# hsiehScalAR/KNODE-Cosserat

Measured on AMD Instinct MI355X. Metric: rod-steps/sec (N=100 segments, batch=1024), higher is better.
Workload: dtype f64

## Files before the change

knode-cosserat_amd/csrc/kr_mso_impl.hpp:

```cpp
#pragma once
#include "kr_ms_impl.hpp"

namespace kr {

constexpr int MSO_B0 = 7 + 17 * (MS_P - 1);
#ifndef KR_MSO_LAG
#define KR_MSO_LAG 1
#endif
constexpr int MSO_LAG = KR_MSO_LAG;
static_assert(MSO_B0 + MS_P <= WAVE, "the verifying lanes must fit beside the forward-difference lanes");

template <typename T, int HS>
__host__ __device__ inline size_t mso_lds_elems(int N) {
  return ms_lds_elems<T, HS>(N, true, false) + 80;
}

__device__ __forceinline__ void wave_sync_lds() {
  __builtin_amdgcn_fence(__ATOMIC_ACQ_REL, "wavefront");
  __builtin_amdgcn_wave_barrier();
}

#define KR_LDS __attribute__((address_space(3)))
template <typename T, int NV>
__device__ __forceinline__ void lds_load_vec(const T* src, T (&v)[NV]) {
  using V = typename Vec16<T>::type;
  constexpr int n = Vec16<T>::n;
  static_assert(NV % n == 0, "vector load needs a multiple of 16 bytes");
  const KR_LDS V* s = (const KR_LDS V*)src;
#pragma unroll
  for (int c = 0; c < NV / n; ++c) {
    const V x = s[c];
#pragma unroll
    for (int e = 0; e < n; ++e) v[c * n + e] = x[e];
  }
}
template <typename T, int NV>
__device__ __forceinline__ void lds_store_vec(T* dst, const T (&v)[NV]) {
  using V = typename Vec16<T>::type;
  constexpr int n = Vec16<T>::n;
  static_assert(NV % n == 0, "vector store needs a multiple of 16 bytes");
  KR_LDS V* d = (KR_LDS V*)dst;
#pragma unroll
  for (int c = 0; c < NV / n; ++c) {
    V x;
#pragma unroll
    for (int e = 0; e < n; ++e) x[e] = v[c * n + e];
    d[c] = x;
  }
}

template <typename U>
__device__ __forceinline__ U own_sgpr(U v) {
  asm volatile("" : "+s"(v));
  return v;
}

template <typename U>
__device__ __forceinline__ U* own_sgpr_global(U* p) {
  uintptr_t v = (uintptr_t)p;
  asm volatile("" : "+s"(v));
  return (U*)(__attribute__((address_space(1))) U*)v;
}

#ifdef KR_MS_STAMPS
struct MsoStats { unsigned long long total = 0, sweeps = 0, merged = 0, quick = 0, chord = 0, rejects = 0, retries = 0, rebuilds = 0, t_sweep = 0, t_alg = 0, t_pred = 0, t_verdict = 0, t_cond = 0, t_fin = 0, t_upd = 0, t_v1 = 0, t_v2 = 0, t_c1 = 0, t_c2 = 0, t_copy = 0; };
#endif

template <typename T, bool DIAG, int HS, int OCC = 1, typename PSRC = RodConst<T>>
__global__ __launch_bounds__(WAVE * MS_WPB, OCC) void mso_sim_kernel(const PSRC Pa, const SimArgs<T> A) {
  extern __shared__ __attribute__((aligned(16))) unsigned char smem_raw[];
  const int N = rod_src_N<T>(Pa);
  const int lane = threadIdx.x & (WAVE - 1);
  const int wv = threadIdx.x / WAVE;
  const int64_t rod = (int64_t)blockIdx.x * MS_WPB + wv;
  if (rod >= A.B) return;
  const auto& Pc = rod_src_row<T>(Pa, rod);
  const size_t rod_elems = (size_t)N * KR_SLOTS;
  T* const a_states = own_sgpr_global(A.states);
  const int64_t a_slot_elems = own_sgpr(A.slot_elems);
  const int a_ring = own_sgpr(A.ring);
  T* const a_tip = own_sgpr_global(A.tip);
  int32_t* const a_status = own_sgpr_global(A.status);
  const int a_residual_test = own_sgpr(A.residual_test), a_predictor = own_sgpr(A.predictor);
  const T hc1 = own_sgpr(A.hc1), hc2 = own_sgpr(A.hc2);
  const int T_steps = own_sgpr((int)A.T_steps);
  const MsLds<T> L = ms_carve<T, HS>(reinterpret_cast<T*>(smem_raw) + (size_t)wv * mso_lds_elems<T, HS>(N), N, true, false);
  T* const Es = L.Es;
  T* const XB = L.XB;
  T* const Tm = L.Tm;
  T* const X0 = L.Xs;
  const ptrdiff_t X_d = (L.c12 + (size_t)N * 12) - L.Xs;
  int xsel = 0;
  T* Xs = X0;
  T* XsB = X0 + X_d;
  T* const EsB = Es + MSO_B0 * MS_YP;
  const MsRole R = ms_role(lane, N);
  const int iv = R.iv, col = R.col;
  const bool isA = lane < MSO_B0;
  const bool isB = lane >= MSO_B0 && lane < MSO_B0 + MS_P;
  const int ib = isB ? lane - MSO_B0 : 0;
  const int s_l = isB ? ms_interval_start(ib, R.sbase, R.srem) : R.s_i;
  const int len_l = isB ? R.sbase + (ib < R.srem ? 1 : 0) : R.len_i;
  ms_cold_fill<T>(rod_src_mem<T>(Pa, rod), L.cold, lane);
  wave_sync();

  auto slot_ptr = [&](int slot) -> T* { return a_states + (int64_t)slot * a_slot_elems + rod * rod_elems; };
  auto state_ptr = [&](int k) -> T* { return slot_ptr(a_ring ? k % 3 : k); };
  T* const lead0 = L.c12;
  const ptrdiff_t lead_d = L.hist - L.c12;
  auto lead_of = [&](int t) -> T* { return lead0 + (ptrdiff_t)(t & 1) * lead_d; };
  auto rebuild = [&](int t) {
    const T* cur = state_ptr(t);
    const T* prv = t > 0 ? state_ptr(t - 1) : (A.prev_init ? A.prev_init + rod * rod_elems : cur);
    T* const lc = lead_of(t);
    T* const lp = lead_of(t - 1);
    for (int j = lane; j < N; j += WAVE) {
      T cv[12], pv[12];
      load_hist_vec<T, 12>(cur + (size_t)j * KR_SLOTS, cv);
      load_hist_vec<T, 12>(prv + (size_t)j * KR_SLOTS, pv);
      lds_store_vec<T, 12>(lc + (size_t)j * 12, cv);
      lds_store_vec<T, 12>(lp + (size_t)j * 12, pv);
    }
    wave_sync();
  };
  const T* ctl = A.ctl + rod * A.T_steps * 4;
  auto load_fc = [&](int t) -> V3<T> {
    V3<T> tf{T(0), T(0), T(0)};
#pragma unroll
    for (int k = 0; k < 4; ++k) {
      const T tt = ctl[(size_t)t * 4 + k];
      tf.x += tt * L.cold[CD_TDIRS + k * 3 + 0];
      tf.y += tt * L.cold[CD_TDIRS + k * 3 + 1];
      tf.z += tt * L.cold[CD_TDIRS + k * 3 + 2];
    }
    return {L.cold[CD_RHOAG] + tf.x, L.cold[CD_RHOAG + 1] + tf.y, L.cold[CD_RHOAG + 2] + tf.z};
  };

  const T* s0 = state_ptr(0);
  const T* sp0 = A.prev_init ? A.prev_init + rod * rod_elems : s0;
  MsPred<T> Q;
  double* img = A.pred_io ? A.pred_io + (size_t)rod * MS_PRED_ROWS * WAVE : nullptr;
  if (img && A.pred_load) ms_pred_load<T>(Q, img, lane);
  else ms_pred_init<T>(Q, lane, R, s0, sp0, A.prev_init != nullptr, a_predictor);
  V3<T> vlast, ulast;
  {
    const T* cl = s0 + (size_t)(N - 1) * KR_SLOTS;
    vlast = {cl[SL_V], cl[SL_V + 1], cl[SL_V + 2]};
    ulast = {cl[SL_U], cl[SL_U + 1], cl[SL_U + 2]};
  }
  const T tol = own_sgpr(A.tol), tolA = own_sgpr(A.tolA), fd_eps = own_sgpr(A.fd_eps);
  const int maxit = own_sgpr(A.maxit);
  T kappa = Q.kappa;
  T Gguess = lane < 6 ? A.G[rod * 6 + lane] : T(0);
  MsStamps stamps;
#ifdef KR_MS_STAMPS
  MsoStats st;
  unsigned long long t_begin, tq;
  KR_STAMP(t_begin);
  tq = t_begin;
#endif

  rebuild(0);

  int tA = 0;
  int rsA = 0;
  bool merged = false;
  int it = 0;
  int order = Q.next_order;
  bool retried = false;
  T dn_prev = T(-1);
  bool have_fac = false, below = false;
  float amp = -1.f;
  T dnB = T(-1);
  float ampB = -1.f;
  bool belowB = false;
  int itB = 0, orderB = 0;
  bool pred_skip = false;
  bool reverify = false;
  int resume_at = T_steps;
  T Xreg[MS_P - 1][2];
#pragma unroll
  for (int g = 0; g < MS_P - 1; ++g) Xreg[g][0] = Xreg[g][1] = T(0);
  V3<T> fcA = load_fc(0), fcB = fcA;
  V3<T> fcN = load_fc(T_steps > 1 ? 1 : 0);
  static_assert(DIAG, "the in-sweep history record assumes diagonal material matrices");
  T hk_a[3], hk_b[3], hk_c[3];
#pragma unroll
  for (int c = 0; c < 3; ++c) {
    hk_a[c] = L.cold[CD_KSEI + 4 * c] * L.cold[CD_KSEV + c];
    hk_b[c] = -L.cold[CD_KSEI + 4 * c] * L.cold[CD_BSE + 4 * c];
    hk_c[c] = -L.cold[CD_KBTI + 4 * c] * L.cold[CD_BBT + 4 * c];
  }

  ms_pred_guess<T>(Q, order, lane, L.cold, Xs);
  wave_sync_lds();
  if (order <= 0 && lane < 6) Xs[0 * MS_YP + 7 + lane] = Gguess;
  wave_sync_lds();

  struct Upd { T updP, updG, xsP, xsG, xsY[MS_P - 1]; };

  while (true) {
    const bool runA = tA < T_steps;
    const int tB = tA - 1;
    T yr[19];
    {
      const T* src = isB ? XsB + ib * MS_YP : Xs + iv * MS_YP;
#pragma unroll
      for (int q = 0; q < 19; ++q) yr[q] = src[q];
    }
    const T hstep = (isA && col > 0) ? fd_eps * fmax(fabs(Xs[iv * MS_YP + (R.comp > 0 ? R.comp : 3)]), T(1)) : T(1);
    int comp = R.comp;
    asm volatile("" : "+v"(comp));
#pragma unroll
    for (int q = 3; q < 19; ++q) yr[q] += q == comp ? hstep : T(0);
    RodState<T> y = rows_to_state(yr);
    const V3<T> fc = isB ? fcB : fcA;
    const int lag = (isA && merged) ? MSO_LAG : 0;
    const bool act = isB ? merged : (isA && runA);
    const int trips = R.lmax + ((merged && runA) ? MSO_LAG : 0);
    T* const out_rod = slot_ptr(rsA);
    auto point_of = [&](int k) -> int {
      const int kk = k - lag;
      return s_l + (kk < 0 ? 0 : (kk < len_l ? kk : len_l - 1));
    };
    const T* const lead_n = lead_of(isB ? tB : tA);
    const T* const lead_o = lead_of(isB ? tB + 1 : tB);
    auto hist_form = [&](const T (&la)[12], const T (&lb)[12]) __attribute__((always_inline)) -> RodHist<T> {
      T raw[12];
#pragma unroll
      for (int c = 0; c < 12; ++c) raw[c] = hc1 * la[c] + hc2 * lb[c];
      RodHist<T> h;
      h.qh = {raw[0], raw[1], raw[2]};
      h.wh = {raw[3], raw[4], raw[5]};
      h.vh = {raw[6], raw[7], raw[8]};
      h.uh = {raw[9], raw[10], raw[11]};
      h.av = {hk_b[0] * raw[6] + hk_a[0], hk_b[1] * raw[7] + hk_a[1], hk_b[2] * raw[8] + hk_a[2]};
      h.au = {hk_c[0] * raw[9], hk_c[1] * raw[10], hk_c[2] * raw[11]};
      return h;
    };
    auto hist_at = [&](int j) __attribute__((always_inline)) -> RodHist<T> {
      T la[12], lb[12];
      lds_load_vec<T, 12>(lead_n + (size_t)j * 12, la);
      lds_load_vec<T, 12>(lead_o + (size_t)j * 12, lb);
      return hist_form(la, lb);
    };
    RodHist<T> hst = hist_at(point_of(0));
    if (!merged) {
      auto fd_point = [&](int j, T dsl) __attribute__((always_inline)) {
        RodState<T> k1;
        V3<T> v, u;
        ode_eval<T, DIAG>(Pc, y, hst, fc, k1, v, u);
        hst = hist_at(j + 1);
        y = state_axpy(y, dsl, k1);
      };
#pragma unroll 2
      for (int t = 0; t < R.sbase; ++t) fd_point(R.s_i + t, Pc.ds);
      if (R.srem) fd_point(R.s_i + (R.len_i > R.sbase ? R.sbase : R.sbase - 1), R.len_i > R.sbase ? Pc.ds : T(0));
    } else {
      const bool lean = a_ring && tB + 4 <= T_steps;
      T* const lead_w = lead_of(tB + 1);
      auto trip = [&](int k, auto full_tag) __attribute__((always_inline)) {
        constexpr bool FULL = decltype(full_tag)::value;
        const int kk = k - lag;
        const bool live = FULL ? act : (act && kk >= 0 && kk < len_l);
        const int j = FULL ? s_l + kk : point_of(k);
        T la[12], lb[12];
        if constexpr (MSO_LAG >= 2) {
          const int jn = FULL ? j + 1 : point_of(k + 1);
          lds_load_vec<T, 12>(lead_n + (size_t)jn * 12, la);
          lds_load_vec<T, 12>(lead_o + (size_t)jn * 12, lb);
        }
        RodState<T> k1;
        V3<T> v, u;
        ode_eval<T, DIAG>(Pc, y, hst, fc, k1, v, u);
        if constexpr (MSO_LAG >= 2) {
          hst = hist_form(la, lb);
          asm volatile("" : "+v"(hst.qh.x), "+v"(hst.qh.y), "+v"(hst.qh.z), "+v"(hst.wh.x), "+v"(hst.wh.y), "+v"(hst.wh.z));
          asm volatile("" : "+v"(hst.vh.x), "+v"(hst.vh.y), "+v"(hst.vh.z), "+v"(hst.uh.x), "+v"(hst.uh.y), "+v"(hst.uh.z));
          asm volatile("" : "+v"(hst.av.x), "+v"(hst.av.y), "+v"(hst.av.z), "+v"(hst.au.x), "+v"(hst.au.y), "+v"(hst.au.z));
        }
        if (isB && live) {
          T rec[KR_SLOTS];
          record_from(y, v, u, rec);
          T lead[12];
#pragma unroll
          for (int c = 0; c < 12; ++c) lead[c] = rec[c];
          if constexpr (FULL) {
            if (!lean) {
              T rest[KR_SLOTS - 12];
#pragma unroll
              for (int c = 0; c < KR_SLOTS - 12; ++c) rest[c] = rec[12 + c];
              store_vec<T, KR_SLOTS - 12>(out_rod + (size_t)j * KR_SLOTS + 12, rest);
            }
          } else {
            store_record(out_rod + (size_t)j * KR_SLOTS, rec);
          }
          lds_store_vec<T, 12>(lead_w + (size_t)j * 12, lead);
        }
        if constexpr (MSO_LAG < 2) hst = hist_at(FULL ? j + 1 : point_of(k + 1));
        const T dsl = live ? Pc.ds : T(0);
        y = state_axpy(y, dsl, k1);
      };
      int k = 0;
      for (; k < MSO_LAG && k < trips; ++k) trip(k, std::false_type{});
#pragma unroll 2
      for (; k < R.sbase; ++k) trip(k, std::true_type{});
      for (; k < trips; ++k) trip(k, std::false_type{});
    }
#ifdef KR_MS_STAMPS
    KR_STAMP_ADD(st.t_sweep, tq);
    st.sweeps += 1;
    if (merged) st.merged += 1;
#endif

    int ln = lane;
    asm volatile("" : "+v"(ln));
    const int kp = ln & 3;
    const int r = 3 + (ln >> 2);
    const bool plane = ln < 3 * (MS_P - 1);
    const int pi = plane ? ln / 3 : 0;
    const int prow = plane ? ln - 3 * pi : 0;
    const bool glane = ln >= WAVE - 6;
    T er[19];
    state_to_rows(y, er);
    T d[6];
    T updY[MS_P - 1];
    T* dYb = XB;
    float dnf = 0.f;
    bool finite = true;
    Upd U;

    auto finish = [&](const T* X, auto base_slot) -> float {
      T* sp = Tm;
      if (kp == 0) {
#pragma unroll
        for (int g = 1; g < MS_P - 1; ++g) dYb[g * MS_YP + r] = updY[g - 1];
      }
      wave_sync_lds();
      if (plane) {
        const int l0 = pi == 0 ? 0 : 7 + 17 * (pi - 1);
        T s = Es[base_slot(pi) * MS_YP + prow] - X[(pi + 1) * MS_YP + prow];
        T av[16], dv[16];
#pragma unroll
        for (int c = 0; c < 16; ++c) {
          const bool use = pi > 0 || c < 6;
          av[c] = use ? Es[(l0 + 1 + c) * MS_YP + prow] : T(0);
          dv[c] = pi > 0 ? dYb[pi * MS_YP + 3 + c] : T(0);
        }
        __builtin_amdgcn_sched_barrier(0);
        T s2 = T(0);
#pragma unroll
        for (int c = 0; c < 16; c += 2) {
          const T da = pi > 0 ? dv[c] : (c < 6 ? d[c < 6 ? c : 0] : T(0));
          const T db = pi > 0 ? dv[c + 1] : (c + 1 < 6 ? d[c + 1 < 6 ? c + 1 : 0] : T(0));
          s = fma(av[c], da, s);
          s2 = fma(av[c + 1], db, s2);
        }
        sp[pi * 3 + prow] = s + s2;
      }
      wave_sync_lds();
      float nf = 0.f;
      U.updP = T(0); U.updG = T(0); U.xsP = T(0); U.xsG = T(0);
      if (plane) {
        U.xsP = X[(pi + 1) * MS_YP + prow];
#pragma unroll
        for (int i = 0; i < MS_P - 1; ++i) {
          const T t = sp[i * 3 + prow];
          U.updP += i <= pi ? t : T(0);
        }
        nf = update_ratio(U.updP, U.xsP);
      }
      if (glane) {
        const int k = ln - (WAVE - 6);
        U.xsG = X[0 * MS_YP + 7 + k];
        U.updG = k == 0 ? d[0] : k == 1 ? d[1] : k == 2 ? d[2] : k == 3 ? d[3] : k == 4 ? d[4] : d[5];
        nf = fmaxf(nf, update_ratio(U.updG, U.xsG));
      }
#pragma unroll
      for (int g = 1; g < MS_P; ++g) {
        U.xsY[g - 1] = T(0);
        if (((g - 1) & 3) == kp) {
          U.xsY[g - 1] = X[g * MS_YP + r];
          nf = fmaxf(nf, update_ratio(updY[g - 1], U.xsY[g - 1]));
        }
      }
      return wave_max_nonneg(nf);
    };
    auto apply = [&](T* X) {
      if (plane) X[(pi + 1) * MS_YP + prow] = U.xsP + U.updP;
      if (glane) X[0 * MS_YP + 7 + (ln - (WAVE - 6))] = U.xsG + U.updG;
#pragma unroll
      for (int g = 1; g < MS_P; ++g)
        if (((g - 1) & 3) == kp) X[g * MS_YP + r] = U.xsY[g - 1] + updY[g - 1];
    };

    if (merged) {
      if (isB) {
#pragma unroll
        for (int q = 0; q < 19; ++q) EsB[ib * MS_YP + q] = er[q];
        if (ib == MS_P - 1) {
          T rec[KR_SLOTS];
          record_from(y, vlast, ulast, rec);
          store_record(out_rod + (size_t)(N - 1) * KR_SLOTS, rec);
          T lead[12];
#pragma unroll
          for (int c = 0; c < 12; ++c) lead[c] = rec[c];
          lds_store_vec<T, 12>(lead_of(tB + 1) + (size_t)(N - 1) * 12, lead);
          if (a_tip) {
            T* tp = a_tip + (rod * T_steps + tB) * 3;
            tp[0] = y.p.x; tp[1] = y.p.y; tp[2] = y.p.z;
          }
        }
      }
      wave_sync_lds();
#ifdef KR_MS_STAMPS
      unsigned long long tv;
      { KR_STAMP(tv); st.t_v1 += tv - tq; }
#endif
      float rn = 0.f;
      if (ln < 3 * MS_YP) {
        const int g = ln / MS_YP, q = ln - MS_YP * g;
        const T x = XsB[(g + 1) * MS_YP + q];
        rn = update_ratio(EsB[g * MS_YP + q] - x, x);
      } else if (ln < 3 * MS_YP + 6) {
        const int k = ln - 3 * MS_YP;
        const T e = EsB[(MS_P - 1) * MS_YP + 7 + k];
        rn = update_ratio(L.cold[CD_FTIP + k] - e, e);
      }
      rn = wave_max_nonneg(rn);
#ifdef KR_MS_STAMPS
      KR_STAMP_ADD(st.t_v2, tv);
#endif
      const float est = ampB * rn;
      bool accepted = a_residual_test != 0 && ampB > 0.f && T(256) * (T)est <= tol;
      float dnv = est;
#ifdef KR_MS_STAMPS
      if (accepted) st.quick += 1;
#endif
      if (!accepted) {
        T* ach = XB;
        T* rt = XB + 4 * MS_YP;
        dYb = XB + MS_YP * 8;
        T areg[MS_P - 1];
        areg[0] = EsB[0 * MS_YP + r] - XsB[1 * MS_YP + r];
        if (kp == 0) ach[1 * MS_YP + r] = areg[0];
        wave_sync_lds();
#pragma unroll
        for (int g = 1; g < MS_P; ++g) {
          const int l0 = 7 + 17 * (g - 1);
          T av[4], xv[4];
#pragma unroll
          for (int cc = 0; cc < 4; ++cc) {
            av[cc] = Es[(l0 + 1 + 4 * kp + cc) * MS_YP + r];
            xv[cc] = ach[g * MS_YP + 3 + 4 * kp + cc];
          }
          const T e0 = EsB[g * MS_YP + r];
          const T ynext = g < MS_P - 1 ? XsB[(g + 1) * MS_YP + r] : T(0);
          T part = fma(av[0], xv[0], av[1] * xv[1]) + fma(av[2], xv[2], av[3] * xv[3]);
          part += quad_xor<0xB1>(part);
          part += quad_xor<0x4E>(part);
          if (g < MS_P - 1) {
            areg[g] = e0 - ynext + part;
            if (kp == 0) ach[(g + 1) * MS_YP + r] = areg[g];
          } else if (kp == 0 && r >= 7 && r < 13) {
            rt[r - 7] = L.cold[CD_FTIP + (r - 7)] - e0 - part;
          }
          wave_sync_lds();
        }
        {
          T rtv[6];
#pragma unroll
          for (int j = 0; j < 6; ++j) rtv[j] = rt[j];
#pragma unroll
          for (int i = 0; i < 6; ++i) {
            T acc = T(0);
#pragma unroll
            for (int j = 0; j < 6; ++j) acc = fma(L.Ti[i * 6 + j], rtv[j], acc);
            d[i] = acc;
          }
        }
        {
          const T dd0 = kp == 0 ? T(0) : kp == 1 ? d[1] : kp == 2 ? d[3] : d[5];
          const T dd1 = kp == 0 ? d[0] : kp == 1 ? d[2] : kp == 2 ? d[4] : T(0);
#pragma unroll
          for (int g = 1; g < MS_P; ++g) {
            T sx = fma(Xreg[g - 1][1], dd1, Xreg[g - 1][0] * dd0);
            sx += quad_xor<0xB1>(sx);
            sx += quad_xor<0x4E>(sx);
            updY[g - 1] = areg[g - 1] + sx;
          }
        }
        dnv = finish(XsB, [](int g) { return MSO_B0 + g; });
        accepted = dnv <= 3.0e38f && (T)dnv <= T(0.5) * tol;
#ifdef KR_MS_STAMPS
        st.chord += 1;
#endif
      }
      if (accepted) {
        {
          const T* const lt = lead_of(tB + 1);
          for (int j = ln; j < N; j += WAVE) {
            T lv[12];
            lds_load_vec<T, 12>(lt + (size_t)j * 12, lv);
            store_vec<T, 12>(out_rod + (size_t)j * KR_SLOTS, lv);
          }
        }
        if (!belowB && dnB > T(0)) {
          const T floor_dn = T(64) * (sizeof(T) == 8 ? T(2.2e-16) : T(1.2e-7));
          const T kq = fmax((T)dnv, floor_dn) * fast_rcp(dnB * dnB);
          kappa = fmin(fmax(kq, T(1e-4)), T(1));
        }
        if (ln == 0 && a_status) a_status[rod * T_steps + tB] = KR_ST_CONVERGED;
        if (ln < 6) Gguess = XsB[0 * MS_YP + 7 + ln];
        pred_skip = false;
        reverify = false;
        merged = false;
        if (!runA) break;
      } else {
#ifdef KR_MS_STAMPS
        st.rejects += 1;
#endif
        const bool ok = dnv <= 3.0e38f;
        if (ok) apply(XsB);
        wave_sync_lds();
        if (ok && !reverify && itB + 2 <= maxit) {
          reverify = true;
          itB += 1;
          dnB = (T)dnv;
          __builtin_amdgcn_fence(__ATOMIC_ACQ_REL, "agent");
          rebuild(tB);
#ifdef KR_MS_STAMPS
          st.rebuilds += 1;
          KR_STAMP_ADD(st.t_alg, tq);
#endif
          continue;
        }
        reverify = false;
        for (int e = ln; e < MS_NE; e += WAVE) Xs[e] = XsB[e];
        tA = tB;
        rsA = a_ring ? (rsA == 0 ? 2 : rsA - 1) : rsA - 1;
        fcN = fcA;
        fcA = fcB;
        order = orderB;
        it = itB;
        dn_prev = ok ? (T)dnv : T(-1);
        have_fac = ok;
        amp = ampB;
        below = false;
        pred_skip = true;
        merged = false;
        __builtin_amdgcn_fence(__ATOMIC_ACQ_REL, "agent");
        rebuild(tA);
#ifdef KR_MS_STAMPS
        st.rebuilds += 1;
        KR_STAMP_ADD(st.t_alg, tq);
#endif
        if (it >= maxit) { resume_at = tA; break; }
        continue;
      }
    }

#ifdef KR_MS_STAMPS
    { unsigned long long t_; KR_STAMP(t_); st.t_verdict += t_ - tq; }
    unsigned long long tq2;
    KR_STAMP(tq2);
#endif
    ++it;
    float res_full;
    {
      const int l0own = iv == 0 ? 0 : 7 + 17 * (iv - 1);
      if (isA && col == 0) {
#pragma unroll
        for (int q = 0; q < 19; ++q) Es[ln * MS_YP + q] = er[q];
      }
      wave_sync_lds();
      res_full = ms_residual_norm<T>(Es, Xs, L.cold, ln);
      if (isA && col > 0) {
        const T ih = fast_rcp(hstep);
        T e0[19];
#pragma unroll
        for (int q = 0; q < 19; ++q) e0[q] = Es[l0own * MS_YP + q];
        __builtin_amdgcn_sched_barrier(0);
#pragma unroll
        for (int q = 0; q < 19; ++q) Es[ln * MS_YP + q] = (er[q] - e0[q]) * ih;
      }
      wave_sync_lds();
    }
#ifdef KR_MS_STAMPS
    unsigned long long tc;
    { KR_STAMP(tc); st.t_c1 += tc - tq2; }
#endif
    dYb = XB;
    {
      const T c0 = Es[0 * MS_YP + r] - Xs[1 * MS_YP + r];
      const T da = Es[(2 * kp) * MS_YP + r];
      const T db = Es[(2 * kp + 1) * MS_YP + r];
      Xreg[0][0] = kp == 0 ? c0 : da;
      Xreg[0][1] = kp == 3 ? T(0) : db;
      store_pair(XB + r * 8 + 2 * kp, Xreg[0][0], Xreg[0][1]);
    }
    wave_sync_lds();
#pragma unroll
    for (int g = 1; g < MS_P; ++g) {
      const T* xcur = XB + ((g - 1) & 1) * (MS_YP * 8);
      T* xnext = XB + (g & 1) * (MS_YP * 8);
      const int l0 = 7 + 17 * (g - 1);
      const T e0 = Es[l0 * MS_YP + r];
      T n0 = T(0), n1 = T(0), n2 = T(0), n3 = T(0);
      if (g < MS_P - 1) {
        const T cg = e0 - Xs[(g + 1) * MS_YP + r];
        n0 = kp == 0 ? cg : T(0);
      }
      {
        T av[16], xa[16], xb[16];
#pragma unroll
        for (int c = 0; c < 16; ++c) {
          av[c] = Es[(l0 + 1 + c) * MS_YP + r];
          load_pair(xcur + (3 + c) * 8 + 2 * kp, xa[c], xb[c]);
        }
        __builtin_amdgcn_sched_barrier(0);
#pragma unroll
        for (int c = 0; c < 16; c += 2) {
          n0 = fma(av[c], xa[c], n0);
          n1 = fma(av[c], xb[c], n1);
          n2 = fma(av[c + 1], xa[c + 1], n2);
          n3 = fma(av[c + 1], xb[c + 1], n3);
        }
        n0 += n2;
        n1 += n3;
      }
      if (g < MS_P - 1) {
        Xreg[g][0] = n0;
        Xreg[g][1] = n1;
        store_pair(xnext + r * 8 + 2 * kp, n0, n1);
      } else if (r >= 7 && r < 13) {
        if (kp == 0) n0 = L.cold[CD_FTIP + (r - 7)] - e0 - n0;
        store_pair(Tm + (r - 7) * 8 + 2 * kp, n0, n1);
      }
      wave_sync_lds();
    }
#ifdef KR_MS_STAMPS
    KR_STAMP_ADD(st.t_c2, tc);
#endif
    {
      T a6[6][7];
      auto fill6 = [&](T (&m)[6][7]) {
#pragma unroll
        for (int i = 0; i < 6; ++i) {
          T row[8];
          load_hist_vec<T, 8>(Tm + i * 8, row);
#pragma unroll
          for (int k = 0; k < 6; ++k) m[i][k] = row[1 + k];
          m[i][6] = ln < 6 ? (ln == i ? T(1) : T(0)) : row[0];
        }
      };
      fill6(a6);
      T x6[6];
      solve6_uniform(a6, x6, fill6);
      if (ln < 6) {
#pragma unroll
        for (int i = 0; i < 6; ++i) L.Ti[i * 6 + ln] = x6[i];
      }
#pragma unroll
      for (int i = 0; i < 6; ++i) d[i] = lane_bcast<6>(x6[i]);
      have_fac = true;
    }
    {
      const T dd0 = kp == 0 ? T(1) : kp == 1 ? d[1] : kp == 2 ? d[3] : d[5];
      const T dd1 = kp == 0 ? d[0] : kp == 1 ? d[2] : kp == 2 ? d[4] : T(0);
#pragma unroll
      for (int g = 1; g < MS_P; ++g) {
        T s = fma(Xreg[g - 1][1], dd1, Xreg[g - 1][0] * dd0);
        s += quad_xor<0xB1>(s);
        s += quad_xor<0x4E>(s);
        updY[g - 1] = s;
      }
    }
#ifdef KR_MS_STAMPS
    KR_STAMP_ADD(st.t_cond, tq2);
#endif
    dnf = finish(Xs, [](int g) { return g == 0 ? 0 : 7 + 17 * (g - 1); });
#ifdef KR_MS_STAMPS
    KR_STAMP_ADD(st.t_fin, tq2);
#endif
    finite = dnf <= 3.0e38f;
    const T dn = (T)dnf;
    if (res_full > 0.f && finite) amp = dnf / res_full;
    if (finite && !below && dn <= tol) {
      below = true;
      if (dn_prev > T(0)) {
        const T floor_dn = T(64) * (sizeof(T) == 8 ? T(2.2e-16) : T(1.2e-7));
        const T kq = fmax(dn, floor_dn) * fast_rcp(dn_prev * dn_prev);
        kappa = fmin(fmax(kq, T(1e-4)), T(1));
      }
    }
    bool next_final = false;
    if (finite) {
      apply(Xs);
      next_final = predict_final<T>(dn, dn_prev, tol, tolA) || (kappa > T(0) && T(4) * kappa * dn * dn <= tol);
      dn_prev = dn;
    }
    wave_sync_lds();
#ifdef KR_MS_STAMPS
    KR_STAMP_ADD(st.t_alg, tq);
#endif
    if (!finite || (it >= maxit && !(next_final && dn <= T(1e-2)))) {
      if (order > 0 && !retried) {
        retried = true;
        order = 0;
        ms_pred_guess<T>(Q, 0, ln, L.cold, Xs);
        wave_sync_lds();
        if (ln < 6) Xs[0 * MS_YP + 7 + ln] = Gguess;
        wave_sync_lds();
        it = 0; dn_prev = T(-1); have_fac = false; amp = -1.f; below = false;
#ifdef KR_MS_STAMPS
        st.retries += 1;
#endif
        continue;
      }
      resume_at = tA;
      break;
    }
    if (next_final && dn <= T(1e-2)) {
      xsel ^= 1;
      Xs = X0 + xsel * X_d;
      XsB = X0 + (1 - xsel) * X_d;
#ifdef KR_MS_STAMPS
      { unsigned long long t_; KR_STAMP(t_); st.t_copy += t_ - tq; }
#endif
      dnB = dn; ampB = amp; belowB = below; itB = it; orderB = order;
      if (!pred_skip) ms_pred_update<T>(Q, order, KR_ST_CONVERGED, a_predictor, lane, XsB, stamps);
#ifdef KR_MS_STAMPS
      { unsigned long long t_; KR_STAMP(t_); st.t_upd += t_ - tq; }
#endif
      tA += 1;
      rsA = a_ring ? (rsA == 2 ? 0 : rsA + 1) : rsA + 1;
      fcB = fcA;
      if (tA < T_steps) {
        fcA = fcN;
        fcN = load_fc(tA + 1 < T_steps ? tA + 1 : tA);
        order = Q.next_order;
        ms_pred_guess<T>(Q, order, lane, L.cold, Xs);
        wave_sync_lds();
        if (order <= 0 && lane < 6) Xs[0 * MS_YP + 7 + lane] = XsB[0 * MS_YP + 7 + lane];
        wave_sync_lds();
      }
      it = 0; retried = false; below = false; dn_prev = T(-1);
      merged = true;
#ifdef KR_MS_STAMPS
      KR_STAMP_ADD(st.t_pred, tq);
#endif
    }
  }

  if (lane < 6) A.G[rod * 6 + lane] = Gguess;
  if (lane == 0 && A.resume) A.resume[rod] = (int32_t)resume_at;
  if (img && (resume_at >= T_steps || !A.resume)) {
    Q.kappa = kappa;
    ms_pred_save<T>(Q, img, lane);
  }
#ifdef KR_MS_STAMPS
  if (lane == 0 && A.dbg) {
    unsigned long long te;
    KR_STAMP(te);
    unsigned long long* dd = A.dbg + rod * 24;
    dd[0] = te - t_begin; dd[1] = st.t_sweep; dd[2] = st.t_alg; dd[3] = st.t_pred; dd[4] = st.sweeps;
    dd[5] = st.merged; dd[6] = st.quick; dd[7] = st.chord; dd[8] = st.rejects; dd[9] = st.retries; dd[10] = st.rebuilds;
    dd[11] = (unsigned long long)resume_at;
    dd[12] = st.t_verdict; dd[13] = st.t_cond; dd[14] = st.t_fin; dd[15] = st.t_upd;
    dd[16] = stamps.a1; dd[17] = stamps.a2; dd[18] = stamps.a3; dd[19] = st.t_v1; dd[20] = st.t_v2; dd[21] = st.t_c1; dd[22] = st.t_c2; dd[23] = st.t_copy;
  }
#endif
}

inline int mso_check_steps(int64_t T_steps) {
  if (T_steps > (int64_t)0x7fffffff) {
    set_error("T_steps = " + std::to_string(T_steps) + ": the overlapped persistent kernel counts steps in 32 bits (T_steps < 2^31)");
    return KR_E_ARG;
  }
  return KR_OK;
}

template <typename T>
int prepare_mso_sim(kr_handle* h, int64_t B) {
  const RodConst<T>& P = consts<T>(h);
  constexpr int HS = hs_phys<T>();
  if (!P.diag || P.N - 1 < 2 * MS_P) return 1;
  const size_t smem = sizeof(T) * mso_lds_elems<T, HS>(P.N) * MS_WPB;
  if (smem > (size_t)h->lds_limit) return 1;
  hipFuncAttributes fa;
  if (sizeof(T) == 4 && B > 1024 && 2 * smem <= (size_t)h->lds_limit) {
    auto k2 = mso_sim_kernel<T, true, HS, 2>;
    KR_HIP(hipFuncGetAttributes(&fa, reinterpret_cast<const void*>(k2)));
    if (int rc_lds_ = dyn_lds(reinterpret_cast<const void*>(k2), smem)) return rc_lds_;
  } else {
    auto k1 = mso_sim_kernel<T, true, HS, 1>;
    KR_HIP(hipFuncGetAttributes(&fa, reinterpret_cast<const void*>(k1)));
    if (int rc_lds_ = dyn_lds(reinterpret_cast<const void*>(k1), smem)) return rc_lds_;
  }
  return KR_OK;
}

template <typename T>
int launch_mso_sim(kr_handle* h, const SimArgs<T>& a, hipStream_t s) {
  const RodConst<T>& P = consts<T>(h);
  constexpr int HS = hs_phys<T>();
  if (!P.diag || P.N - 1 < 2 * MS_P) return 1;
  const size_t smem = sizeof(T) * mso_lds_elems<T, HS>(P.N) * MS_WPB;
  if (smem > (size_t)h->lds_limit) return 1;
  if (int rc_steps_ = mso_check_steps(a.T_steps)) return rc_steps_;
  const dim3 grid((unsigned)((a.B + MS_WPB - 1) / MS_WPB)), block(WAVE * MS_WPB);
  if constexpr (sizeof(T) == 4) {
    if (a.B > 1024 && 2 * smem <= (size_t)h->lds_limit) {
      auto kern2 = mso_sim_kernel<T, true, HS, 2>;
      if (int rc_lds_ = dyn_lds(reinterpret_cast<const void*>(kern2), smem)) return rc_lds_;
      hipLaunchKernelGGL(kern2, grid, block, smem, s, P, a);
      KR_HIP(hipGetLastError());
      return KR_OK;
    }
  }
  auto kern = mso_sim_kernel<T, true, HS, 1>;
  if (int rc_lds_ = dyn_lds(reinterpret_cast<const void*>(kern), smem)) return rc_lds_;
  hipLaunchKernelGGL(kern, grid, block, smem, s, P, a);
  KR_HIP(hipGetLastError());
  return KR_OK;
}

}
```

Baseline: 43.78 million.

## Split history blend to prefetch older lead early and specialise lean sweep loop

The history interpolation is split so the older-step term is loaded from LDS and scaled before the ODE evaluation, while the newest term is loaded after and combined with an fma. The intent is to hide LDS latency behind the ODE evaluation. The full-trip loop is manually unrolled by two and specialised at compile time on the lean flag, so the per-trip branch on skipping global stores disappears. In the merged path the end-state rows are written to Es early, which removes a second store and a wave sync before the residual. The extra live registers and scheduling barriers could cost occupancy.

```diff
diff --git a/knode-cosserat_amd/csrc/kr_mso_impl.hpp b/knode-cosserat_amd/csrc/kr_mso_impl.hpp
--- a/knode-cosserat_amd/csrc/kr_mso_impl.hpp
+++ b/knode-cosserat_amd/csrc/kr_mso_impl.hpp
@@ -225,10 +225,14 @@
     };
     const T* const lead_n = lead_of(isB ? tB : tA);
     const T* const lead_o = lead_of(isB ? tB + 1 : tB);
-    auto hist_form = [&](const T (&la)[12], const T (&lb)[12]) __attribute__((always_inline)) -> RodHist<T> {
+    auto hist_older = [&](const T (&lb)[12], T (&pb)[12]) __attribute__((always_inline)) {
+#pragma unroll
+      for (int c = 0; c < 12; ++c) pb[c] = hc2 * lb[c];
+    };
+    auto hist_newest = [&](const T (&la)[12], const T (&pb)[12]) __attribute__((always_inline)) -> RodHist<T> {
       T raw[12];
 #pragma unroll
-      for (int c = 0; c < 12; ++c) raw[c] = hc1 * la[c] + hc2 * lb[c];
+      for (int c = 0; c < 12; ++c) raw[c] = fma(hc1, la[c], pb[c]);
       RodHist<T> h;
       h.qh = {raw[0], raw[1], raw[2]};
       h.wh = {raw[3], raw[4], raw[5]};
@@ -237,6 +241,11 @@
       h.av = {hk_b[0] * raw[6] + hk_a[0], hk_b[1] * raw[7] + hk_a[1], hk_b[2] * raw[8] + hk_a[2]};
       h.au = {hk_c[0] * raw[9], hk_c[1] * raw[10], hk_c[2] * raw[11]};
       return h;
+    };
+    auto hist_form = [&](const T (&la)[12], const T (&lb)[12]) __attribute__((always_inline)) -> RodHist<T> {
+      T pb[12];
+      hist_older(lb, pb);
+      return hist_newest(la, pb);
     };
     auto hist_at = [&](int j) __attribute__((always_inline)) -> RodHist<T> {
       T la[12], lb[12];
@@ -259,16 +268,23 @@
     } else {
       const bool lean = a_ring && tB + 4 <= T_steps;
       T* const lead_w = lead_of(tB + 1);
-      auto trip = [&](int k, auto full_tag) __attribute__((always_inline)) {
+      auto trip = [&](int k, auto full_tag, auto lean_tag) __attribute__((always_inline)) {
         constexpr bool FULL = decltype(full_tag)::value;
+        constexpr bool LEAN = decltype(lean_tag)::value;
         const int kk = k - lag;
         const bool live = FULL ? act : (act && kk >= 0 && kk < len_l);
         const int j = FULL ? s_l + kk : point_of(k);
-        T la[12], lb[12];
+        const int eo = j * 12;
+        const int en = FULL ? eo + 12 : point_of(k + 1) * 12;
+        T la[12], lb[12], pb[12];
         if constexpr (MSO_LAG >= 2) {
-          const int jn = FULL ? j + 1 : point_of(k + 1);
-          lds_load_vec<T, 12>(lead_n + (size_t)jn * 12, la);
-          lds_load_vec<T, 12>(lead_o + (size_t)jn * 12, lb);
+          lds_load_vec<T, 12>(lead_n + en, la);
+          lds_load_vec<T, 12>(lead_o + en, lb);
+        } else {
+          lds_load_vec<T, 12>(lead_o + en, lb);
+#ifdef KR_MSO_PROBE_EARLY_READS
+          if constexpr (FULL) lds_load_vec<T, 12>(lead_n + en, la);
+#endif
         }
         RodState<T> k1;
         V3<T> v, u;
@@ -278,6 +294,10 @@
           asm volatile("" : "+v"(hst.qh.x), "+v"(hst.qh.y), "+v"(hst.qh.z), "+v"(hst.wh.x), "+v"(hst.wh.y), "+v"(hst.wh.z));
           asm volatile("" : "+v"(hst.vh.x), "+v"(hst.vh.y), "+v"(hst.vh.z), "+v"(hst.uh.x), "+v"(hst.uh.y), "+v"(hst.uh.z));
           asm volatile("" : "+v"(hst.av.x), "+v"(hst.av.y), "+v"(hst.av.z), "+v"(hst.au.x), "+v"(hst.au.y), "+v"(hst.au.z));
+        } else {
+          hist_older(lb, pb);
+          asm volatile("" : "+v"(pb[0]), "+v"(pb[1]), "+v"(pb[2]), "+v"(pb[3]), "+v"(pb[4]), "+v"(pb[5]), "+v"(pb[6]), "+v"(pb[7]),
+                            "+v"(pb[8]), "+v"(pb[9]), "+v"(pb[10]), "+v"(pb[11]));
         }
         if (isB && live) {
           T rec[KR_SLOTS];
@@ -286,26 +306,48 @@
 #pragma unroll
           for (int c = 0; c < 12; ++c) lead[c] = rec[c];
           if constexpr (FULL) {
-            if (!lean) {
+            if constexpr (!LEAN) {
               T rest[KR_SLOTS - 12];
 #pragma unroll
               for (int c = 0; c < KR_SLOTS - 12; ++c) rest[c] = rec[12 + c];
               store_vec<T, KR_SLOTS - 12>(out_rod + (size_t)j * KR_SLOTS + 12, rest);
             }
           } else {
-            store_record(out_rod + (size_t)j * KR_SLOTS, rec);
+            if (!(lean && k >= R.sbase)) store_record(out_rod + (size_t)j * KR_SLOTS, rec);
           }
-          lds_store_vec<T, 12>(lead_w + (size_t)j * 12, lead);
-        }
-        if constexpr (MSO_LAG < 2) hst = hist_at(FULL ? j + 1 : point_of(k + 1));
+          lds_store_vec<T, 12>(lead_w + eo, lead);
+        }
+        if constexpr (MSO_LAG < 2) {
+#ifdef KR_MSO_PROBE_EARLY_READS
+          if constexpr (!FULL)
+#endif
+          lds_load_vec<T, 12>(lead_n + en, la);
+          if constexpr (OCC == 1) __builtin_amdgcn_sched_barrier(0);
+        }
         const T dsl = live ? Pc.ds : T(0);
         y = state_axpy(y, dsl, k1);
+        if constexpr (MSO_LAG < 2) {
+          asm volatile("" : "+v"(pb[0]), "+v"(pb[1]), "+v"(pb[2]), "+v"(pb[3]), "+v"(pb[4]), "+v"(pb[5]), "+v"(pb[6]), "+v"(pb[7]),
+                            "+v"(pb[8]), "+v"(pb[9]), "+v"(pb[10]), "+v"(pb[11]), "+v"(y.p.z), "+v"(y.h3), "+v"(y.n.z), "+v"(y.m.z),
+                            "+v"(y.q.z), "+v"(y.w.z));
+          hst = hist_newest(la, pb);
+        }
       };
       int k = 0;
-      for (; k < MSO_LAG && k < trips; ++k) trip(k, std::false_type{});
-#pragma unroll 2
-      for (; k < R.sbase; ++k) trip(k, std::true_type{});
-      for (; k < trips; ++k) trip(k, std::false_type{});
+      for (; k < MSO_LAG && k < trips; ++k) trip(k, std::false_type{}, std::false_type{});
+      auto full_trips = [&](auto lean_tag) __attribute__((always_inline)) {
+        for (; k + 1 < R.sbase; k += 2) {
+          trip(k, std::true_type{}, lean_tag);
+          trip(k + 1, std::true_type{}, lean_tag);
+        }
+        if (k < R.sbase) {
+          trip(k, std::true_type{}, lean_tag);
+          ++k;
+        }
+      };
+      if (lean) full_trips(std::true_type{});
+      else full_trips(std::false_type{});
+      for (; k < trips; ++k) trip(k, std::false_type{}, std::false_type{});
     }
 #ifdef KR_MS_STAMPS
     KR_STAMP_ADD(st.t_sweep, tq);
@@ -394,10 +436,13 @@
         if (((g - 1) & 3) == kp) X[g * MS_YP + r] = U.xsY[g - 1] + updY[g - 1];
     };
 
+    const bool es_stored = merged;
     if (merged) {
+      if (isB || (isA && col == 0)) {
+#pragma unroll
+        for (int q = 0; q < 19; ++q) Es[ln * MS_YP + q] = er[q];
+      }
       if (isB) {
-#pragma unroll
-        for (int q = 0; q < 19; ++q) EsB[ib * MS_YP + q] = er[q];
         if (ib == MS_P - 1) {
           T rec[KR_SLOTS];
           record_from(y, vlast, ulast, rec);
@@ -569,11 +614,13 @@
     float res_full;
     {
       const int l0own = iv == 0 ? 0 : 7 + 17 * (iv - 1);
-      if (isA && col == 0) {
-#pragma unroll
-        for (int q = 0; q < 19; ++q) Es[ln * MS_YP + q] = er[q];
-      }
-      wave_sync_lds();
+      if (!es_stored) {
+        if (isA && col == 0) {
+#pragma unroll
+          for (int q = 0; q < 19; ++q) Es[ln * MS_YP + q] = er[q];
+        }
+        wave_sync_lds();
+      }
       res_full = ms_residual_norm<T>(Es, Xs, L.cold, ln);
       if (isA && col > 0) {
         const T ih = fast_rcp(hstep);
```

Result: faster. 46.45 million (median of 6 runs) (+6.1%).
